# JingwenWang95/DSP-SLAM

Hardware: NVIDIA H100
Metric: object-recons/sec (2048 pts, 10 GN iters) (higher is better)
Workload: dtype f16x3-split (fp32 accumulate)

## Files before the change

### dsp_slam_b200/csrc/dspgn_tc.cuh

```cuda
#pragma once
#include <cuda_fp16.h>
#include <string>
#include <vector>
#include "dspgn_simt.cuh"
#include "dspgn_solve.cuh"

namespace dspgn {

constexpr int kTcThreads = 384;
constexpr int kTcEpiThreads = 256;
constexpr int kTcStages = 4;
constexpr int kTcStageBytes = 16384;
constexpr int kTcAloBytes = 32768;
constexpr int kTcProducerRegs = 40, kTcConsumerRegs = 232;
static_assert(128 * kTcProducerRegs + 256 * kTcConsumerRegs <= 384 * 168, "setmaxnreg budget exceeds the CTA's registers");

__host__ __device__ constexpr int tc_mma_n(int n) { return n <= 80 ? 80 : (n <= 192 ? 192 : 256); }
__host__ __device__ constexpr int tc_pad_k_steps(int k_steps) { return (k_steps + 3) / 4 * 4; }

__device__ __forceinline__ uint32_t smem_u32(const void* p) { return (uint32_t)__cvta_generic_to_shared(p); }

__device__ __forceinline__ void mbar_init(uint64_t* bar, uint32_t count) {
  asm volatile("mbarrier.init.shared::cta.b64 [%0], %1;" ::"r"(smem_u32(bar)), "r"(count) : "memory");
}
__device__ __forceinline__ void mbar_arrive(uint32_t bar) {
  asm volatile("mbarrier.arrive.shared::cta.b64 _, [%0];" ::"r"(bar) : "memory");
}
__device__ __forceinline__ void mbar_expect_tx(uint64_t* bar, uint32_t bytes) {
  asm volatile("mbarrier.arrive.expect_tx.shared::cta.b64 _, [%0], %1;" ::"r"(smem_u32(bar)), "r"(bytes) : "memory");
}
__device__ __forceinline__ void mbar_wait(uint32_t bar, uint32_t parity) {
  asm volatile(
      "{\n\t"
      ".reg .pred p;\n\t"
      "WAIT_LOOP:\n\t"
      "mbarrier.try_wait.parity.shared::cta.b64 p, [%0], %1;\n\t"
      "@p bra DONE;\n\t"
      "bra WAIT_LOOP;\n\t"
      "DONE:\n\t"
      "}" ::"r"(bar), "r"(parity) : "memory");
}
__device__ __forceinline__ void mbar_wait(uint64_t* bar, uint32_t parity) { mbar_wait(smem_u32(bar), parity); }
__device__ __forceinline__ void fence_barrier_init() { asm volatile("fence.mbarrier_init.release.cluster;" ::: "memory"); }

__device__ __forceinline__ void bulk_g2s(void* smem_dst, const void* gmem_src, uint32_t bytes, uint64_t* bar) {
  asm volatile("cp.async.bulk.shared::cluster.global.mbarrier::complete_tx::bytes [%0], [%1], %2, [%3];" ::"r"(smem_u32(smem_dst)),
               "l"(gmem_src), "r"(bytes), "r"(smem_u32(bar)) : "memory");
}

__device__ __forceinline__ void fence_proxy_async() { asm volatile("fence.proxy.async.shared::cta;" ::: "memory"); }
__device__ __forceinline__ void wg_fence() { asm volatile("wgmma.fence.sync.aligned;" ::: "memory"); }
__device__ __forceinline__ void wg_commit() { asm volatile("wgmma.commit_group.sync.aligned;" ::: "memory"); }
__device__ __forceinline__ void wg_wait0() { asm volatile("wgmma.wait_group.sync.aligned 0;" ::: "memory"); }
__device__ __forceinline__ void wg_wait1() { asm volatile("wgmma.wait_group.sync.aligned 1;" ::: "memory"); }
template <int REGS> __device__ __forceinline__ void setmaxnreg_inc() { asm volatile("setmaxnreg.inc.sync.aligned.u32 %0;" ::"n"(REGS)); }
template <int REGS> __device__ __forceinline__ void setmaxnreg_dec() { asm volatile("setmaxnreg.dec.sync.aligned.u32 %0;" ::"n"(REGS)); }
__device__ __forceinline__ void wg_bar_sync(int g) { asm volatile("bar.sync %0, 128;" ::"r"(3 + g) : "memory"); }

#define DSPGN_D8(o) "+f"(d[o + 0]), "+f"(d[o + 1]), "+f"(d[o + 2]), "+f"(d[o + 3]), "+f"(d[o + 4]), "+f"(d[o + 5]), "+f"(d[o + 6]), "+f"(d[o + 7])
#define DSPGN_D128                                                                                                    \
  DSPGN_D8(0), DSPGN_D8(8), DSPGN_D8(16), DSPGN_D8(24), DSPGN_D8(32), DSPGN_D8(40), DSPGN_D8(48), DSPGN_D8(56),         \
      DSPGN_D8(64), DSPGN_D8(72), DSPGN_D8(80), DSPGN_D8(88), DSPGN_D8(96), DSPGN_D8(104), DSPGN_D8(112), DSPGN_D8(120)
#define DSPGN_D96                                                                                                     \
  DSPGN_D8(0), DSPGN_D8(8), DSPGN_D8(16), DSPGN_D8(24), DSPGN_D8(32), DSPGN_D8(40), DSPGN_D8(48), DSPGN_D8(56),         \
      DSPGN_D8(64), DSPGN_D8(72), DSPGN_D8(80), DSPGN_D8(88)
#define DSPGN_D40 DSPGN_D8(0), DSPGN_D8(8), DSPGN_D8(16), DSPGN_D8(24), DSPGN_D8(32)
#define DSPGN_ACC_OPS128 "{%0, %1, %2, %3, %4, %5, %6, %7, %8, %9, %10, %11, %12, %13, %14, %15, %16, %17, %18, %19, %20, %21, %22, %23, %24, %25, %26, %27, %28, %29, %30, %31, %32, %33, %34, %35, %36, %37, %38, %39, %40, %41, %42, %43, %44, %45, %46, %47, %48, %49, %50, %51, %52, %53, %54, %55, %56, %57, %58, %59, %60, %61, %62, %63, %64, %65, %66, %67, %68, %69, %70, %71, %72, %73, %74, %75, %76, %77, %78, %79, %80, %81, %82, %83, %84, %85, %86, %87, %88, %89, %90, %91, %92, %93, %94, %95, %96, %97, %98, %99, %100, %101, %102, %103, %104, %105, %106, %107, %108, %109, %110, %111, %112, %113, %114, %115, %116, %117, %118, %119, %120, %121, %122, %123, %124, %125, %126, %127}, "
#define DSPGN_ACC_OPS96 "{%0, %1, %2, %3, %4, %5, %6, %7, %8, %9, %10, %11, %12, %13, %14, %15, %16, %17, %18, %19, %20, %21, %22, %23, %24, %25, %26, %27, %28, %29, %30, %31, %32, %33, %34, %35, %36, %37, %38, %39, %40, %41, %42, %43, %44, %45, %46, %47, %48, %49, %50, %51, %52, %53, %54, %55, %56, %57, %58, %59, %60, %61, %62, %63, %64, %65, %66, %67, %68, %69, %70, %71, %72, %73, %74, %75, %76, %77, %78, %79, %80, %81, %82, %83, %84, %85, %86, %87, %88, %89, %90, %91, %92, %93, %94, %95}, "
#define DSPGN_ACC_OPS40 "{%0, %1, %2, %3, %4, %5, %6, %7, %8, %9, %10, %11, %12, %13, %14, %15, %16, %17, %18, %19, %20, %21, %22, %23, %24, %25, %26, %27, %28, %29, %30, %31, %32, %33, %34, %35, %36, %37, %38, %39}, "

template <int N> struct Wgmma;
#define DSPGN_WGMMA(N, DREGS, OPS, R0, R1, R2, R3, R4, R5, S0, S1, S2)                                          \
  template <> struct Wgmma<N> {                                                                                 \
    static __device__ __forceinline__ void rs(float (&d)[128], uint32_t a0, uint32_t a1, uint32_t a2, uint32_t a3, \
                                              uint64_t b_desc) {                                                \
      asm volatile("{\n\t.reg .pred p;\n\tsetp.ne.b32 p, %" #R5 ", 0;\n\t"                                       \
                   "wgmma.mma_async.sync.aligned.m64n" #N "k16.f32.f16.f16 " OPS                                 \
                   "{%" #R0 ", %" #R1 ", %" #R2 ", %" #R3 "}, %" #R4 ", p, 1, 1, 0;\n\t}"                         \
                   : DREGS                                                                                      \
                   : "r"(a0), "r"(a1), "r"(a2), "r"(a3), "l"(b_desc), "r"(1)                                    \
                   : "memory");                                                                                 \
    }                                                                                                           \
    static __device__ __forceinline__ void ss(float (&d)[128], uint64_t a_desc, uint64_t b_desc) {              \
      asm volatile("{\n\t.reg .pred p;\n\tsetp.ne.b32 p, %" #S2 ", 0;\n\t"                                       \
                   "wgmma.mma_async.sync.aligned.m64n" #N "k16.f32.f16.f16 " OPS                                 \
                   "%" #S0 ", %" #S1 ", p, 1, 1, 0, 0;\n\t}"                                                     \
                   : DREGS                                                                                      \
                   : "l"(a_desc), "l"(b_desc), "r"(1)                                                           \
                   : "memory");                                                                                 \
    }                                                                                                           \
  };
DSPGN_WGMMA(256, DSPGN_D128, DSPGN_ACC_OPS128, 128, 129, 130, 131, 132, 133, 128, 129, 130)
DSPGN_WGMMA(192, DSPGN_D96, DSPGN_ACC_OPS96, 96, 97, 98, 99, 100, 101, 96, 97, 98)
DSPGN_WGMMA(80, DSPGN_D40, DSPGN_ACC_OPS40, 40, 41, 42, 43, 44, 45, 40, 41, 42)
#undef DSPGN_WGMMA

__device__ __forceinline__ void epi_bar_sync() { asm volatile("bar.sync 1, 256;" ::: "memory"); }

enum ProbeSlot {
  PR_WFULL, PR_WGWAIT, PR_GEMM, PR_EPI, PR_PROLOGUE, PR_JTJ, PR_TILE_END, PR_SOLVE, PR_FIFO, PR_LOOP, PR_TILES, PR_SOLVES,
  PR_WEMPTY, PR_POP, PR_PROD_LOOP, kProbeSlots = 16
};
constexpr int kProbeCtas = 256;
#ifdef DSPGN_STALL_PROBE
__device__ unsigned long long g_stall_probe[kProbeCtas * 3 * kProbeSlots];
__device__ __forceinline__ void probe_add(int slot, unsigned long long v) {
  if ((threadIdx.x & 127) == 0 && blockIdx.x < kProbeCtas)
    atomicAdd(&g_stall_probe[(blockIdx.x * 3 + (threadIdx.x >> 7)) * kProbeSlots + slot], v);
}
#define DSPGN_PROBE_T(t0) const long long t0 = clock64()
#define DSPGN_PROBE_ADD(slot, t0) probe_add(slot, (unsigned long long)(clock64() - (t0)))
#define DSPGN_PROBE_COUNT(slot) probe_add(slot, 1ull)
#else
#define DSPGN_PROBE_T(t0)
#define DSPGN_PROBE_ADD(slot, t0)
#define DSPGN_PROBE_COUNT(slot)
#endif

__device__ __forceinline__ uint64_t make_desc(uint32_t smem_addr) {
  uint64_t d = 0;
  d |= (uint64_t)((smem_addr >> 4) & 0x3FFF);
  d |= (uint64_t)1 << 16;
  d |= (uint64_t)64 << 32;
  d |= (uint64_t)1 << 62;
  return d;
}
__device__ __forceinline__ uint64_t make_desc_w(uint32_t smem_addr) {
  uint64_t d = 0;
  d |= (uint64_t)((smem_addr >> 4) & 0x3FFF);
  d |= (uint64_t)1 << 16;
  d |= (uint64_t)32 << 32;
  d |= (uint64_t)2 << 62;
  return d;
}

__device__ __forceinline__ void split_pack(float a, float b, uint32_t& hi, uint32_t& lo) {
  __half2 h = __floats2half2_rn(a, b);
  float2 back = __half22float2(h);
  __half2 l = __floats2half2_rn(a - back.x, b - back.y);
  hi = *reinterpret_cast<uint32_t*>(&h);
  lo = *reinterpret_cast<uint32_t*>(&l);
}

constexpr int kJpStride = 76;
struct TcSmemTail {
  float Jp[kTcRows * kJpStride];
  uint32_t maskw[8 * 4 * kTcEpiThreads];
  float bias[9 * kHid];
  float wlast[kHid];
  float w0x[3 * kHid];
  float zs[kMaxCode + 16];
  float xr[3 * kTcRows];
  float rr[kTcRows], rsc[kTcRows];
  float yrow[kTcRows], scr[kTcRows];
  int prefix[kMaxObjScan + 1];
  int warp_tmp[32];
  uint64_t w_full[kTcStages], w_empty[kTcStages];
  int cur_class;
  int fifo[4]; int fifo_pub; int epi_seq; int last_flag;
  TcPlan plans[DSPGN_MAX_CLASSES];
  BatchDev ctx_b; MegaArgs ctx_q; SolveArgs ctx_sv;
  int push_base, push_nF, push_nS, push_o;
  float ost[16]; int ost_rows;
};
constexpr size_t kTcSmemBytes = 1024 + (size_t)kTcStages * kTcStageBytes + 2 * (size_t)kTcAloBytes + sizeof(TcSmemTail);
static_assert(kTcSmemBytes <= 227 * 1024, "tensor-core engine shared memory exceeds the 227 KB per block of sm_90");
static_assert(offsetof(TcSmemTail, bias) % 8 == 0, "the hidden-layer epilogue reads bias column pairs as float2");

__device__ __forceinline__ int frag_col(int e, int q) { return 8 * (e >> 2) + 2 * q + (e & 1); }
__device__ __forceinline__ int opaque_int(int v) {
  int r;
  asm volatile("mov.b32 %0, %1;" : "=r"(r) : "r"(v));
  return r;
}

__device__ __forceinline__ void store_operand(const float (&v)[128], uint32_t (&ah)[64], unsigned char* alo, int rl, int q, int grp) {
#pragma unroll
  for (int t = 0; t < 16; ++t) {
#pragma unroll
    for (int h = 0; h < 4; ++h) {
      uint32_t hi, lo;
      split_pack(v[8 * t + 2 * h], v[8 * t + 2 * h + 1], hi, lo);
      ah[4 * t + h] = hi;
      const int row = rl + 8 * (h & 1), kk = 16 * t + 8 * (h >> 1) + 2 * q;
      const int off = (kk >> 6) * 8192 + row * 128 + ((((kk & 63) >> 3) ^ (row & 7)) << 4) + (kk & 7) * 2;
      *reinterpret_cast<uint32_t*>(alo + off) = lo;
    }
  }
  fence_proxy_async();
  wg_bar_sync(grp);
}

__device__ __forceinline__ void release_stage(uint32_t w_empty, int s) {
  __syncwarp();
  if ((threadIdx.x & 31) == 0) mbar_arrive(w_empty + 8u * s);
}

template <int N>
__device__ __forceinline__ void wg_gemm(float (&acc)[128], const uint32_t (&ah)[64], uint32_t alo, uint32_t ring,
                                        uint32_t bars, uint32_t& phase, int nch) {
  static_assert(kTcStages == 4, "one ring lap per K chunk");
  const uint32_t w_full = bars, w_empty = bars + 8u * kTcStages;
#pragma unroll
  for (int i = 0; i < 128; ++i) acc[i] = 0.f;
#pragma unroll
  for (int c = 0; c < 4; ++c) {
    if (c < nch) {
      const uint32_t ph = phase ^ (uint32_t)(c & 1);
#pragma unroll
      for (int s = 0; s < kTcStages; ++s) {
        DSPGN_PROBE_T(tf);
        mbar_wait(w_full + 8u * s, ph);
        DSPGN_PROBE_ADD(PR_WFULL, tf);
        wg_fence();
        const uint32_t bw = ring + (uint32_t)s * kTcStageBytes;
#pragma unroll
        for (int k = 0; k < 2; ++k) {
          const int t = 4 * c + 2 * (s & 1) + k;
          const uint64_t bd = make_desc_w(bw + 32u * k);
          Wgmma<N>::rs(acc, ah[4 * t], ah[4 * t + 1], ah[4 * t + 2], ah[4 * t + 3], bd);
          if (s < 2) Wgmma<N>::ss(acc, make_desc(alo + 8192u * c + 32u * (t & 3)), bd);
        }
        wg_commit();
        if (s == 1) {
          DSPGN_PROBE_T(tw);
          wg_wait1();
          DSPGN_PROBE_ADD(PR_WGWAIT, tw);
          release_stage(w_empty, 0);
          if (c > 0) release_stage(w_empty, 3);
        } else if (s == 3) {
          DSPGN_PROBE_T(tw);
          wg_wait1();
          DSPGN_PROBE_ADD(PR_WGWAIT, tw);
          release_stage(w_empty, 1);
          release_stage(w_empty, 2);
        }
      }
    }
  }
  DSPGN_PROBE_T(tw);
  wg_wait0();
  DSPGN_PROBE_ADD(PR_WGWAIT, tw);
  release_stage(w_empty, 3);
  phase ^= (uint32_t)(nch & 1);
}

__device__ __forceinline__ void produce_step(const unsigned char* src, int nch, uint32_t img_bytes, unsigned char* ring,
                                             uint64_t* w_full, uint64_t* w_empty, uint32_t& phase) {
  for (int c = 0; c < nch; ++c) {
    for (int s = 0; s < kTcStages; ++s) {
      DSPGN_PROBE_T(te);
      mbar_wait(&w_empty[s], phase ^ 1);
      DSPGN_PROBE_ADD(PR_WEMPTY, te);
      mbar_expect_tx(&w_full[s], img_bytes);
      bulk_g2s(ring + (size_t)s * kTcStageBytes, src + (size_t)(kTcStages * c + s) * img_bytes, img_bytes, &w_full[s]);
    }
    phase ^= 1;
  }
}

struct TileRef { int o, row0, slot, mode, tile; };

constexpr unsigned long long kMegaTimeoutNs = 30ull * 1000ull * 1000ull * 1000ull;
__device__ inline int mega_pop(const MegaArgs& q, int n_obj) {
  for (;;) {
    const int t = atomicAdd(&q.ctr->head, 1);
    if (t >= q.q_cap) return -1;
    unsigned long long t0 = 0;
    int item = kItemNop;
    for (unsigned spins = 0;; ++spins) {
      const int v = ldv(q.q_flag + t);
      if (v != 0) { __threadfence(); item = v - 1; break; }
      if (ldv(&q.ctr->done_objects) >= n_obj || ldv(&q.ctr->abort_flag) != 0) return -1;
      __nanosleep(256);
      if ((spins & 1023u) == 1023u) {
        const unsigned long long now = globaltimer_ns();
        if (t0 == 0) t0 = now;
        else if (now - t0 > kMegaTimeoutNs) { atomicExch(&q.ctr->abort_flag, 1); return -1; }
      }
    }
    if (item != kItemNop) return item;
  }
}

template <int SCHED>
__device__ __forceinline__ bool tile_at(const BatchDev& b, const TermArgs& a, TcSmemTail& S, int seq, int total_tiles, TileRef& t) {
  constexpr bool MEGA = SCHED != 0;
  if (!MEGA) {
    const int tile = blockIdx.x + seq * gridDim.x;
    if (tile >= total_tiles) return false;
    t.o = find_object(S.prefix, b.n_obj, tile);
    t.tile = tile - S.prefix[t.o];
    t.row0 = t.tile * kTcRows;
    t.slot = tile;
    t.mode = a.mode;
    return true;
  } else {
    volatile int* pub = &S.fifo_pub;
    while (*pub <= seq) __nanosleep(64);
    const int item = reinterpret_cast<volatile int*>(S.fifo)[seq & 3];
    if (item < 0) return false;
    t.o = (item >> kItemObjShift) & kItemObjMask;
    t.mode = (SCHED == 1) ? MODE_SDF : (item >> kItemKindShift);
    const int j = item & kItemTileMask;
    t.tile = j;
    t.row0 = j * kTcRows;
    t.slot = (t.mode == MODE_BAND) ? a.tile_base_r[t.o] + j : (t.mode == MODE_SDF ? a.tile_base[t.o] + j : 0);
    return true;
  }
}

__device__ __forceinline__ int mega_rows(const BatchDev& b, const MegaArgs& q, const ObjMeta& M, int o, int mode) {
  if (mode == MODE_SDF) return M.n_pts;
  if (mode == MODE_BAND) return ldv(b.band_m + o);
  if (q.vpre != nullptr) return ldv(q.vpre + vpre_base(M, o) + M.n_rays) >> 7;
  return M.n_rays * b.D;
}

__device__ inline void mega_push(const MegaArgs& q, int kind, int o, int n) {
  if (n <= 0) return;
  const int base = atomicAdd(&q.ctr->tail, n);
  __threadfence();
  for (int j = 0; j < n; ++j) *reinterpret_cast<volatile int*>(q.q_flag + base + j) = make_item(kind, o, j) + 1;
}

__device__ __noinline__ void mega_solve_and_advance(TcSmemTail& S, int o, int tid) {
  const BatchDev& b = S.ctx_b;
  const MegaArgs& q = S.ctx_q;
  const SolveArgs& sv = S.ctx_sv;
  __threadfence();
  SolveSmem& SM = *reinterpret_cast<SolveSmem*>(S.Jp);
  const int it = ldv(q.obj_iter + o);
  const bool render = q.render && b.state[o].mode == DSPGN_MODE_JOINT;
  if (tid == 0) log_event(q.log, ev_desc(EV_SOLVE_BEGIN, 0, o, it));
  const int fin = solve_object<true>(b, sv, q.log, o, tid, SM, it + 1 >= b.state[o].n_iter);
  epi_bar_sync();
  int vh = -1;
  if (!fin && render && q.vpre != nullptr) {
    const ObjMeta M = b.meta[o];
    if (M.n_rays > 0) vh = valid_sample_ranges<true>(M, b.state[o], b.rays, b.D, q.vpre + vpre_base(M, o), tid, kTcEpiThreads, S.warp_tmp);
  }
  if (tid == 0) {
    log_event(q.log, ev_desc(EV_SOLVE_END, 0, o, it));
// ... 86 lines not shown
        for (int s = 0; s < ns; ++s)
          produce_step(blob + plan.step[s].w_off, plan.step[s].k_steps / 4, 64u * (uint32_t)plan.step[s].n_mma, ring, S.w_full,
                       S.w_empty, phase);
      }
      DSPGN_PROBE_ADD(PR_PROD_LOOP, tloop);
    }
  } else {
    setmaxnreg_inc<kTcConsumerRegs>();
    const int grp = warp >> 2;
    const int r = tid & 127;
    const int qd = lane & 3;
    const int rl = 16 * (warp & 3) + (lane >> 2);
    const int rowA = 64 * grp + rl, rowB = rowA + 8;
    unsigned char* const alo = ring + (size_t)kTcStages * kTcStageBytes + (size_t)grp * kTcAloBytes;
    const uint32_t alo_s = smem_u32(alo), ring_s = smem_u32(ring);
    uint32_t phase = 0;
    float acc[128];
    uint32_t ah[64];
    DSPGN_PROBE_T(tloop);
    for (int seq = 0;; ++seq) {
      TileRef tr;
      DSPGN_PROBE_T(tq);
      if (!tile_at<SCHED>(b, a, S, seq, total_tiles, tr)) break;
      DSPGN_PROBE_ADD(PR_FIFO, tq);
      DSPGN_PROBE_T(tpro);
      if (MEGA && tid == 0) { *reinterpret_cast<volatile int*>(&S.epi_seq) = seq + 1; log_event(q.log, ev_desc(EV_TILE_BEGIN, tr.mode, tr.o, tr.tile)); }
      if (RENDER && tr.mode == kKindScan) {
        const int o = tr.o;
        scan_chunk(b, sv.prm.th, q.vpre, q.seg_cnt, o, tr.tile, tid);
        __threadfence();
        epi_bar_sync();
        if (tid == 0) {
          log_event(q.log, ev_desc(EV_TILE_END, tr.mode, o, tr.tile));
          *reinterpret_cast<volatile int*>(&S.last_flag) = (atomicSub(q.scan_left + o, 1) == 1) ? 1 : 0;
        }
        epi_bar_sync();
        int act = *reinterpret_cast<volatile int*>(&S.last_flag);
        if (act == 1) {
          __threadfence();
          scan_prefix(b, q.seg_cnt, q.seg_prefix, o, tid, S.warp_tmp);
          epi_bar_sync();
          if (tid == 0) {
            __threadfence();
            atomicAdd(&q.ctr->valid_rows_total, (unsigned long long)ldv(b.V_count + o));
            const int m = ldv(b.band_m + o);
            const int ntB = (m + kTcRows - 1) / kTcRows;
            atomicAdd(&q.ctr->band_rows_total, m);
            const int left = atomicAdd(q.pending + o, ntB - 1) + ntB - 1;
            mega_push(q, MODE_BAND, o, ntB);
            *reinterpret_cast<volatile int*>(&S.last_flag) = (left == 0) ? 2 : 0;
          }
          epi_bar_sync();
          act = *reinterpret_cast<volatile int*>(&S.last_flag);
        } else act = 0;
        if (act == 2) mega_solve_and_advance(S, o, tid);
        continue;
      }
      const int o = tr.o, row0 = tr.row0, tile = tr.slot, mode = tr.mode;
      const ObjMeta M = b.meta[o];
      const ObjState& ost = b.state[o];
      const DecoderDev& dec = b.decs[M.class_id];
      const TcPlan& plan = S.plans[M.class_id];
      const int L = dec.L, in0 = dec.in0, n_lin = dec.n_lin;
      const bool has_skip = dec.latent_in >= 0;
      const bool grid_mode = !MEGA && mode == MODE_GRIDFWD;
      const bool fwd_only = (mode == MODE_RAYFWD || mode == MODE_PTSFWD || grid_mode);
      const int ns = fwd_only ? plan.n_fwd : plan.n_steps;
      const float huber_b = term_huber(a, mode, ost.mode, (RENDER && mode == MODE_BAND) ? a.huber_b1 : a.huber_b);
      float* const part = (RENDER && mode == MODE_BAND) ? a.part_r : a.part;
      if (tid < 12) S.ost[tid] = ldv(&ost.T_oc[tid]);
      else if (tid < 16) S.ost[tid] = ldv(&ost.dmin + (tid - 12));
      const bool pts_mode = (mode == MODE_SDF || mode == MODE_PTSFWD || grid_mode);
      if (MEGA && !pts_mode && tid == 16) S.ost_rows = mega_rows(b, q, M, o, mode);

      if (S.cur_class != M.class_id) {
        for (int i = tid; i < n_lin * kHid; i += kTcEpiThreads) S.bias[i] = dec.bias[i / kHid][i % kHid];
        for (int i = tid; i < kHid; i += kTcEpiThreads) S.wlast[i] = dec.w_last[i];
        const float* __restrict__ w0g = dec.Wf[0] + (size_t)L * kHid;
        for (int i = tid; i < 3 * kHid; i += kTcEpiThreads) S.w0x[i] = w0g[i];
      }
      if (tid < kMaxCode + 16) S.zs[tid] = (tid < L) ? ldv(&ost.z[tid]) : 0.f;
      S.bias[tid] = ldv(&ost.zb0[tid]);
      const uint8_t* mask_in; uint8_t* mask_out;
      cut_masks(a, ost.mode, (MEGA && a.cut_iter >= 0) ? ldv(q.obj_iter + o) : a.iter, mask_in, mask_out);
      const int* segp = nullptr;
      int nseg = 0;
      const bool compact = RENDER && mode == MODE_RAYFWD && q.vpre != nullptr;
      if (compact) {
        int* sp = reinterpret_cast<int*>(S.Jp);
        const int* gp = q.vpre + vpre_base(M, o);
        for (int i = tid; i <= M.n_rays; i += kTcEpiThreads) sp[i] = __ldcg(gp + i);
        segp = sp;
      }
      if (RENDER && mode == MODE_BAND) {
        nseg = (M.n_rays + kSegRays - 1) / kSegRays;
        int* sp = reinterpret_cast<int*>(S.Jp);
        const int* gp = q.seg_prefix + seg_base(M, o);
        for (int i = tid; i <= nseg; i += kTcEpiThreads) sp[i] = __ldcg(gp + i);
        segp = sp;
      }
      int nrows = 0;
      float p0 = 0.f, p1 = 0.f, p2 = 0.f, sc = 0.f;
      if (pts_mode) {
        nrows = min(kTcRows, (MEGA ? M.n_pts : term_rows(b, a, o)) - row0);
        if (r < nrows) {
          const float* pq = grid_mode ? a.grid + 3 * (size_t)(row0 + r) : b.pts + 3 * (size_t)(M.pts_off + row0 + r);
          p0 = pq[0]; p1 = pq[1]; p2 = pq[2];
          sc = (grid_mode || mask_in == nullptr || ldv(mask_in + M.pts_off + row0 + r)) ? 1.f : 0.f;
        }
      }
      epi_bar_sync();
      float Toc[12];
#pragma unroll
      for (int i = 0; i < 12; ++i) Toc[i] = S.ost[i];
      if (!pts_mode) nrows = min(kTcRows, (MEGA ? S.ost_rows : term_rows(b, a, o)) - row0);
      float x0 = 0.f, x1 = 0.f, x2 = 0.f, res_in = 0.f;
      if (r < nrows) {
        const int rr_ = row0 + r;
        if (grid_mode) {
          x0 = p0; x1 = p1; x2 = p2;
        } else if (pts_mode) {
          xform_point(Toc, p0, p1, p2, x0, x1, x2);
        } else if (mode == MODE_BAND) {
          size_t sidx = (size_t)M.smp_off + rr_;
          if (RENDER) {
            int lo = 0, hi = nseg;
            while (hi - lo > 1) { const int mid = (lo + hi) >> 1; if (segp[mid] <= rr_) lo = mid; else hi = mid; }
            sidx = (size_t)M.smp_off + (size_t)lo * kSegRays * b.D + (size_t)(rr_ - segp[lo]);
          }
          x0 = __ldcg(b.band_x + 3 * sidx); x1 = __ldcg(b.band_x + 3 * sidx + 1); x2 = __ldcg(b.band_x + 3 * sidx + 2);
          sc = __ldcg(b.band_s + sidx); res_in = __ldcg(b.band_r + sidx);
        } else {
          int ray = rr_ / b.D, j = rr_ - ray * b.D;
          if (compact) {
            int lo = 0, hi = M.n_rays;
            while (hi - lo > 1) { const int mid = (lo + hi) >> 1; if ((segp[mid] >> 7) <= rr_) lo = mid; else hi = mid; }
            ray = lo; j = (segp[lo] & 127) + (rr_ - (segp[lo] >> 7));
          }
          const float* rq = b.rays + 3 * (size_t)(M.ray_off + ray);
          const float d = lin_depth(S.ost[12], S.ost[13], S.ost[14], j, b.D);
          xform_point(Toc, __fmul_rn(rq[0], d), __fmul_rn(rq[1], d), __fmul_rn(rq[2], d), x0, x1, x2);
          sc = inside_unit_sphere(x0, x1, x2) ? 1.f : 0.f;
        }
      }
      if (grp == 0) { S.xr[r] = x0; S.xr[kTcRows + r] = x1; S.xr[2 * kTcRows + r] = x2; S.scr[r] = sc; }
      epi_bar_sync();
      if (tid == 0) S.cur_class = M.class_id;

      auto inp = [&](int i, int row) -> float {
        const int j = i - L;
        return (j < 0) ? S.zs[i] : ((unsigned)j < 3u ? S.xr[j * kTcRows + row] : 0.f);
      };
      uint32_t* const maskw = S.maskw + tid;

      {
        const int kk = plan.step[0].k_steps * 16;
        const int n0out = dec.out_dim[0];
        const float* w0x = S.w0x;
        const float xa0 = S.xr[rowA], xa1 = S.xr[kTcRows + rowA], xa2 = S.xr[2 * kTcRows + rowA];
        const float xb0 = S.xr[rowB], xb1 = S.xr[kTcRows + rowB], xb2 = S.xr[2 * kTcRows + rowB];
        const int qs = opaque_int(qd);
        uint32_t mw[4] = {0u, 0u, 0u, 0u};
#pragma unroll
        for (int e = 0; e < 128; ++e) {
          const int c = frag_col(e, qs);
          const bool hb = (e & 2) != 0;
          float w = S.bias[c];
          w = fmaf(w0x[c], hb ? xb0 : xa0, w);
          w = fmaf(w0x[kHid + c], hb ? xb1 : xa1, w);
          w = fmaf(w0x[2 * kHid + c], hb ? xb2 : xa2, w);
          const bool on = (c < kk) && (c < n0out) && (w > 0.f);
          mw[e >> 5] |= (on ? 1u : 0u) << (e & 31);
          acc[e] = on ? w : 0.f;
        }
#pragma unroll
        for (int w = 0; w < 4; ++w) maskw[w * kTcEpiThreads] = mw[w];
        store_operand(acc, ah, alo, rl, qd, grp);
      }
      DSPGN_PROBE_ADD(PR_PROLOGUE, tpro);
      DSPGN_PROBE_COUNT(PR_TILES);

      float yv = 0.f;
      for (int s = 0; s < ns; ++s) {
        const TcStep st = plan.step[s];
        const bool more = (s + 1 < ns);
        const int k_next = more ? plan.step[s + 1].k_steps * 16 : 0;
        const int nm = st.n_mma;
        if (MEGA && tid == 0 && s == 0) log_event(q.log, ev_desc(EV_FIRST_MMA, tr.mode, tr.o, tr.tile));
        const int nch = st.k_steps / 4;
        DSPGN_PROBE_T(tg);
        if (nm == 80) wg_gemm<80>(acc, ah, alo_s, ring_s, smem_u32(S.w_full), phase, nch);
        else if (nm == 192) wg_gemm<192>(acc, ah, alo_s, ring_s, smem_u32(S.w_full), phase, nch);
        else wg_gemm<256>(acc, ah, alo_s, ring_s, smem_u32(S.w_full), phase, nch);
        DSPGN_PROBE_ADD(PR_GEMM, tg);
        DSPGN_PROBE_T(tepi);
        wg_bar_sync(grp);
        const int qs = opaque_int(qd);

        if (st.kind == TK_FWD_PENULT) {
          const float* bb = S.bias + st.layer * kHid;
          float pa = 0.f, pb = 0.f;
          uint32_t mw[4] = {0u, 0u, 0u, 0u};
#pragma unroll
          for (int e = 0; e < 128; ++e) {
            const int c = frag_col(e, qs);
            if (c < nm) {
              const float w = acc[e] + bb[c];
              mw[e >> 5] |= (w > 0.f ? 1u : 0u) << (e & 31);
              if (e & 2) pb = fmaf(fmaxf(w, 0.f), S.wlast[c], pb);
              else pa = fmaf(fmaxf(w, 0.f), S.wlast[c], pa);
            }
          }
#pragma unroll
          for (int w = 0; w < 4; ++w) maskw[(4 * st.layer + w) * kTcEpiThreads] = mw[w];
          pa += __shfl_xor_sync(0xffffffffu, pa, 1);
          pb += __shfl_xor_sync(0xffffffffu, pb, 1);
          pa += __shfl_xor_sync(0xffffffffu, pa, 2);
          pb += __shfl_xor_sync(0xffffffffu, pb, 2);
          const float blast = S.bias[(st.layer + 1) * kHid];
          const float ya = tanhf(pa + blast), yb = tanhf(pb + blast);
          if (qd == 0) { S.yrow[rowA] = ya; S.yrow[rowB] = yb; }
          epi_bar_sync();
          yv = S.yrow[r];
          if (fwd_only) {
            if (grp == 0 && r < nrows) {
              const size_t base = (mode == MODE_RAYFWD) ? (size_t)M.smp_off
                                  : (grid_mode ? (size_t)a.grid_slot[o] * a.grid_rows : (size_t)M.pts_off);
              b.sdf[base + row0 + r] = (sc != 0.f) ? yv : INFINITY;
            }
            if (!RENDER && mode == MODE_RAYFWD) {
              const unsigned bal = __ballot_sync(0xffffffffu, grp == 0 && r < nrows && sc != 0.f);
              if (lane == 0 && bal) atomicAdd(b.V_count + o, __popc(bal));
            }
          }
          if (more) {
            const float ga = 1.f - ya * ya, gb = 1.f - yb * yb;
#pragma unroll
            for (int e = 0; e < 128; ++e) {
              const int c = frag_col(e, qs);
              acc[e] = ((mw[e >> 5] >> (e & 31)) & 1u) ? ((e & 2) ? gb : ga) * S.wlast[c] : 0.f;
            }
            store_operand(acc, ah, alo, rl, qd, grp);
          }
        } else if (st.kind == TK_FWD_HIDDEN) {
          const float* bb = S.bias + st.layer * kHid;
          uint32_t mw[4] = {0u, 0u, 0u, 0u};
          if (SCHED == 1 && st.cat_off < 0) {
#pragma unroll
            for (int j = 0; j < 32; ++j) {
              const float2 bj = *reinterpret_cast<const float2*>(bb + 8 * j + 2 * qs);
#pragma unroll
              for (int h = 0; h < 4; ++h) {
                const int e = 4 * j + h, c = frag_col(e, qs);
                const float w = acc[e] + ((h & 1) ? bj.y : bj.x);
                const bool live = c < nm;
                mw[e >> 5] |= ((live && w > 0.f) ? 1u : 0u) << (e & 31);
                acc[e] = (live && c < k_next) ? fmaxf(w, 0.f) : 0.f;
              }
            }
          } else {
#pragma unroll
            for (int e = 0; e < 128; ++e) {
              const int c = frag_col(e, qs);
              float t = 0.f;
              if (c < nm) {
                const float w = acc[e] + bb[c];
                mw[e >> 5] |= (w > 0.f ? 1u : 0u) << (e & 31);
                t = fmaxf(w, 0.f);
              }
              if (st.cat_off >= 0 && c >= st.cat_off) t = inp(c - st.cat_off, (e & 2) ? rowB : rowA);
              acc[e] = (c < k_next) ? t : 0.f;
            }
          }
#pragma unroll
          for (int w = 0; w < 4; ++w) maskw[(4 * st.layer + w) * kTcEpiThreads] = mw[w];
          store_operand(acc, ah, alo, rl, qd, grp);
        } else if (st.kind == TK_BWD_MID) {
          uint32_t mw[4];
#pragma unroll
          for (int w = 0; w < 4; ++w) mw[w] = maskw[(4 * st.mask_layer + w) * kTcEpiThreads];
          if (SCHED == 1 && st.cat_off < 0) {
#pragma unroll
            for (int e = 0; e < 128; ++e) {
              const int c = frag_col(e, qs);
              const bool on = c < nm && c < k_next && ((mw[e >> 5] >> (e & 31)) & 1u);
              acc[e] = on ? acc[e] : 0.f;
            }
          } else {
#pragma unroll
            for (int e = 0; e < 128; ++e) {
              const int c = frag_col(e, qs);
              float t = 0.f;
              if (c < nm) {
                const float v = acc[e];
                t = ((mw[e >> 5] >> (e & 31)) & 1u) ? v : 0.f;
                if (st.cat_off >= 0 && c >= st.cat_off) {
                  const int ii = c - st.cat_off;
                  if (ii < in0) S.Jp[((e & 2) ? rowB : rowA) * kJpStride + ((ii < L) ? ii : (kMaxCode + ii - L))] = v;
                  t = 0.f;
                }
              }
              acc[e] = (c < k_next) ? t : 0.f;
            }
          }
          if (more) store_operand(acc, ah, alo, rl, qd, grp);
        } else {
#pragma unroll
          for (int e = 0; e < 128; ++e) {
            const int c = frag_col(e, qs);
            if (c < nm && c < in0) {
              const int row = (e & 2) ? rowB : rowA;
              float* pj = S.Jp + row * kJpStride + ((c < L) ? c : (kMaxCode + c - L));
              float g = acc[e];
              if (has_skip) g += *pj;
              *pj = g * S.scr[row];
            }
          }
        }
        if (!more || st.kind == TK_BWD_FIRST) {
#pragma unroll
          for (int i = 0; i < 64; ++i) ah[i] = 0u;
        }
        DSPGN_PROBE_ADD(PR_EPI, tepi);
      }
      DSPGN_PROBE_T(tjtj);
      if (!fwd_only) {
      epi_bar_sync();
      if (grp == 0) {
        float* jr = S.Jp + r * kJpStride;
        for (int i = L; i < kMaxCode; ++i) jr[i] = 0.f;
        const float g0 = jr[kMaxCode], g1 = jr[kMaxCode + 1], g2 = jr[kMaxCode + 2];
        jr[kMaxCode + 3] = x1 * g2 - x2 * g1;
        jr[kMaxCode + 4] = x2 * g0 - x0 * g2;
        jr[kMaxCode + 5] = x0 * g1 - x1 * g0;
        jr[kMaxCode + 6] = (ost.mode == DSPGN_MODE_POSE) ? 0.f : (g0 * x0 + g1 * x1 + g2 * x2);
        jr[kMaxCode + 7] = 0.f;
        float res = (mode == MODE_SDF) ? yv : res_in;
        if (sc == 0.f && (mode == MODE_SDF || r >= nrows)) res = 0.f;
        if (mask_out != nullptr && mode == MODE_SDF && r < nrows)
          mask_out[M.pts_off + row0 + r] = (sc != 0.f && fabsf(res) <= 0.05f) ? 1 : 0;
        S.rr[r] = huber_weight(fabsf(res), huber_b) * res;
        S.rsc[r] = (mode == MODE_SDF) ? sc : (r < nrows ? 1.f : 0.f);
        if (a.dbg_J != nullptr && o == a.dbg_obj && mode == MODE_SDF && r < nrows) a.dbg_res[row0 + r] = res;
      }
      epi_bar_sync();
      if (a.dbg_J != nullptr && o == a.dbg_obj && mode == MODE_SDF) {
        const int P = a.dbg_P, npose = (ost.mode == DSPGN_MODE_POSE) ? 6 : 7;
        for (int idx = tid; idx < nrows * P; idx += kTcEpiThreads) {
          const int p = idx / P, c = idx - p * P;
          const int ci = (c < npose) ? (kMaxCode + c) : (c - npose);
          a.dbg_J[(size_t)(row0 + p) * P + c] = S.Jp[p * kJpStride + ci];
        }
      }
      float* accp = part + (size_t)tile * kAccStride;
      if (tid < 171) {
        int bi = 0, rem = tid;
        while (rem >= 18 - bi) { rem -= 18 - bi; ++bi; }
        const int bj = bi + rem;
        float h[4][4];
#pragma unroll
        for (int u = 0; u < 4; ++u)
#pragma unroll
          for (int v = 0; v < 4; ++v) h[u][v] = 0.f;
        const float* pa = S.Jp + 4 * bi;
        const float* pb = S.Jp + 4 * bj;
#pragma unroll 4
        for (int p = 0; p < kTcRows; ++p) {
          const float4 A4 = *reinterpret_cast<const float4*>(pa + p * kJpStride);
          const float4 B4 = *reinterpret_cast<const float4*>(pb + p * kJpStride);
          const float av[4] = {A4.x, A4.y, A4.z, A4.w}, bv[4] = {B4.x, B4.y, B4.z, B4.w};
#pragma unroll
          for (int u = 0; u < 4; ++u)
#pragma unroll
            for (int v = 0; v < 4; ++v) h[u][v] = fmaf(av[u], bv[v], h[u][v]);
        }
#pragma unroll
        for (int u = 0; u < 4; ++u)
#pragma unroll
          for (int v = 0; v < 4; ++v) {
            const int rI = 4 * bi + u, cI = 4 * bj + v;
            if (cI >= rI && cI < kMaxCode + 7) accp[tri_index(rI, cI)] = h[u][v];
          }
      } else if (tid < 171 + kMaxCode + 7) {
        const int c = tid - 171;
        float sacc = 0.f;
        for (int p = 0; p < kTcRows; ++p) sacc = fmaf(S.Jp[p * kJpStride + c], S.rr[p], sacc);
        accp[kAccB + c] = sacc;
      } else if (tid >= 248) {
        const int k = tid - 248;
        float sacc = 0.f, n = 0.f;
        for (int p = 16 * k; p < 16 * k + 16; ++p) { sacc = fmaf(S.rr[p], S.rr[p], sacc); n += S.rsc[p]; }
#pragma unroll
        for (int d = 1; d < 8; d <<= 1) {
          sacc += __shfl_down_sync(0xff000000u, sacc, d);
          n += __shfl_down_sync(0xff000000u, n, d);
        }
        if (k == 0) { accp[kAccLoss] = sacc; accp[kAccLoss + 1] = n; }
      }
      }
      DSPGN_PROBE_ADD(PR_JTJ, tjtj);
      if (MEGA) {
        DSPGN_PROBE_T(tend);
        __threadfence();
        epi_bar_sync();
        if (tid == 0) {
          log_event(q.log, ev_desc(EV_TILE_END, mode, o, tr.tile));
          int act = 0;
          if (RENDER && mode == MODE_RAYFWD) { if (atomicSub(q.ray_left + o, 1) == 1) act = 1; }
          else if (atomicSub(q.pending + o, 1) == 1) act = 2;
          *reinterpret_cast<volatile int*>(&S.last_flag) = act;
        }
        epi_bar_sync();
        int act = *reinterpret_cast<volatile int*>(&S.last_flag);
        if (RENDER && act == 1) {
          if (tid == 0) {
            const int nch = (M.n_rays + kScanChunkRays - 1) / kScanChunkRays;
            *reinterpret_cast<volatile int*>(q.scan_left + o) = nch;
            __threadfence();
            mega_push(q, kKindScan, o, nch);
          }
        }
        DSPGN_PROBE_ADD(PR_TILE_END, tend);
        if (act == 2) {
          DSPGN_PROBE_T(tsv);
          mega_solve_and_advance(S, o, tid);
          DSPGN_PROBE_ADD(PR_SOLVE, tsv);
          DSPGN_PROBE_COUNT(PR_SOLVES);
        }
      }
    }
    DSPGN_PROBE_ADD(PR_LOOP, tloop);
  }
}

__global__ void __launch_bounds__(kTcThreads, 1) k_decoder_tc(BatchDev b, TermArgs a) {
  tc_body<0>(b, a, MegaArgs{}, SolveArgs{});
}
__global__ void __launch_bounds__(kTcThreads, 1) k_gn_persistent(BatchDev b, TermArgs a, MegaArgs q, SolveArgs sv) {
  tc_body<1>(b, a, q, sv);
}
__global__ void __launch_bounds__(kTcThreads, 1) k_gn_persistent_render(BatchDev b, TermArgs a, MegaArgs q, SolveArgs sv) {
  tc_body<2>(b, a, q, sv);
}

constexpr size_t kTcSelftestSmem = 1024 + (size_t)kTcStages * kTcStageBytes + 2 * (size_t)kTcAloBytes + 64;
__global__ void __launch_bounds__(kTcThreads, 1) k_tc_selftest(const float* __restrict__ A, int lda, const unsigned char* __restrict__ blob,
                                                               int n_mma, int k_steps, float* __restrict__ D) {
  extern __shared__ unsigned char st_raw[];
  unsigned char* ring = st_raw + ((1024u - (smem_u32(st_raw) & 1023u)) & 1023u);
  uint64_t* bars = reinterpret_cast<uint64_t*>(ring + (size_t)kTcStages * kTcStageBytes + 2 * (size_t)kTcAloBytes);
  uint64_t* w_full = bars;
  uint64_t* w_empty = bars + kTcStages;
  const int tid = threadIdx.x, warp = tid >> 5, lane = tid & 31;
  if (tid == 0) {
    for (int i = 0; i < kTcStages; ++i) { mbar_init(&w_full[i], 1); mbar_init(&w_empty[i], 8); }
    fence_barrier_init();
  }
  __syncthreads();
  const int n_img = tc_mma_n(n_mma), nch = tc_pad_k_steps(k_steps) / 4;
  uint32_t phase = 0;
  if (warp >= 8) {
    setmaxnreg_dec<kTcProducerRegs>();
    if (warp == 8 && lane == 0) produce_step(blob, nch, 64u * (uint32_t)n_img, ring, w_full, w_empty, phase);
    return;
  }
  setmaxnreg_inc<kTcConsumerRegs>();
  const int grp = warp >> 2, qd = lane & 3, rl = 16 * (warp & 3) + (lane >> 2);
  const int rowA = 64 * grp + rl, rowB = rowA + 8;
  unsigned char* alo = ring + (size_t)kTcStages * kTcStageBytes + (size_t)grp * kTcAloBytes;
  float acc[128];
// ... 137 lines not shown
```

Baseline: 4042.

## Specialize tensor-core epilogues and store low operand halves with stmatrix

For the SCHED==1 path, the low fp16 split halves are written to shared memory with stmatrix.x4 instead of per-element 32-bit stores. The per-kind epilogue loops (hidden forward, concat, skip gradient, backward mid, first backward) are rewritten to work on 8-column groups, with compile-time NM/KNEXT specializations for common widths, and the concat/skip layers now also take the fast path. The goal is fewer instructions, less predicate work and fewer shared-store transactions in the epilogue. The cost is more code paths and more register pressure, and the stmatrix swizzle has to match the existing layout exactly. Extra probe slots are also added for timing.

```diff
diff --git a/dsp_slam_b200/csrc/dspgn_tc.cuh b/dsp_slam_b200/csrc/dspgn_tc.cuh
--- a/dsp_slam_b200/csrc/dspgn_tc.cuh
+++ b/dsp_slam_b200/csrc/dspgn_tc.cuh
@@ -99,8 +99,9 @@
 
 enum ProbeSlot {
   PR_WFULL, PR_WGWAIT, PR_GEMM, PR_EPI, PR_PROLOGUE, PR_JTJ, PR_TILE_END, PR_SOLVE, PR_FIFO, PR_LOOP, PR_TILES, PR_SOLVES,
-  PR_WEMPTY, PR_POP, PR_PROD_LOOP, kProbeSlots = 16
+  PR_WEMPTY, PR_POP, PR_PROD_LOOP, PR_EPI_ENTRY, PR_EPI_KIND, kProbeSlots = PR_EPI_KIND + 3 * 6
 };
+enum EpiKind { EK_FWD, EK_FWD_CAT, EK_PENULT, EK_BWD, EK_BWD_SKIP, EK_BWD_FIRST };
 constexpr int kProbeCtas = 256;
 #ifdef DSPGN_STALL_PROBE
 __device__ unsigned long long g_stall_probe[kProbeCtas * 3 * kProbeSlots];
@@ -111,10 +112,12 @@
 #define DSPGN_PROBE_T(t0) const long long t0 = clock64()
 #define DSPGN_PROBE_ADD(slot, t0) probe_add(slot, (unsigned long long)(clock64() - (t0)))
 #define DSPGN_PROBE_COUNT(slot) probe_add(slot, 1ull)
+#define DSPGN_PROBE_ADD_IF(cond, slot, t0) do { if (cond) DSPGN_PROBE_ADD(slot, t0); } while (0)
 #else
 #define DSPGN_PROBE_T(t0)
 #define DSPGN_PROBE_ADD(slot, t0)
 #define DSPGN_PROBE_COUNT(slot)
+#define DSPGN_PROBE_ADD_IF(cond, slot, t0)
 #endif
 
 __device__ __forceinline__ uint64_t make_desc(uint32_t smem_addr) {
@@ -174,7 +177,9 @@
   return r;
 }
 
-__device__ __forceinline__ void store_operand(const float (&v)[128], uint32_t (&ah)[64], unsigned char* alo, int rl, int q, int grp) {
+__device__ __forceinline__ void store_operand(const float (&v)[128], uint32_t (&ah)[64], unsigned char* alo, int rl, int q, int grp,
+                                              int pslot = -1) {
+  DSPGN_PROBE_T(ts);
 #pragma unroll
   for (int t = 0; t < 16; ++t) {
 #pragma unroll
@@ -187,8 +192,109 @@
       *reinterpret_cast<uint32_t*>(alo + off) = lo;
     }
   }
+  DSPGN_PROBE_ADD_IF(pslot >= 0, pslot + 1, ts);
+  DSPGN_PROBE_T(tf);
   fence_proxy_async();
   wg_bar_sync(grp);
+  DSPGN_PROBE_ADD_IF(pslot >= 0, pslot + 2, tf);
+}
+
+__device__ __forceinline__ void store_operand_stsm(const float (&v)[128], uint32_t (&ah)[64], uint32_t alo, int grp, int pslot = -1) {
+  DSPGN_PROBE_T(ts);
+  const int lane = threadIdx.x & 31;
+  const int srow = 16 * ((threadIdx.x >> 5) & 3) + (lane & 7) + 8 * ((lane >> 3) & 1);
+  const uint32_t base = alo + 128u * (uint32_t)srow;
+  const uint32_t xo = (uint32_t)(((lane >> 4) & 1) ^ (lane & 7)) << 4;
+#pragma unroll
+  for (int t = 0; t < 16; ++t) {
+    uint32_t lo[4];
+#pragma unroll
+    for (int h = 0; h < 4; ++h) split_pack(v[8 * t + 2 * h], v[8 * t + 2 * h + 1], ah[4 * t + h], lo[h]);
+    const uint32_t addr = base + 8192u * (uint32_t)(t >> 2) + (xo ^ (32u * (uint32_t)(t & 3)));
+    asm volatile("stmatrix.sync.aligned.m8n8.x4.shared.b16 [%0], {%1, %2, %3, %4};" ::"r"(addr), "r"(lo[0]), "r"(lo[1]),
+                 "r"(lo[2]), "r"(lo[3]) : "memory");
+  }
+  DSPGN_PROBE_ADD_IF(pslot >= 0, pslot + 1, ts);
+  DSPGN_PROBE_T(tf);
+  fence_proxy_async();
+  wg_bar_sync(grp);
+  DSPGN_PROBE_ADD_IF(pslot >= 0, pslot + 2, tf);
+}
+
+template <int NM, int KNEXT>
+__device__ __forceinline__ void epi_fwd_hidden(float (&acc)[128], uint32_t (&mw)[4], const float* bb, int qs, int nm, int k_next) {
+#pragma unroll
+  for (int j = 0; j < 32; ++j) {
+    const bool live = 8 * j < (NM ? NM : nm), nxt = 8 * j < (KNEXT ? KNEXT : k_next);
+    const float2 bj = *reinterpret_cast<const float2*>(bb + 8 * j + 2 * qs);
+#pragma unroll
+    for (int h = 0; h < 4; ++h) {
+      const int e = 4 * j + h;
+      const float w = acc[e] + ((h & 1) ? bj.y : bj.x);
+      mw[e >> 5] |= ((live && w > 0.f) ? 1u : 0u) << (e & 31);
+      acc[e] = (live && nxt) ? fmaxf(w, 0.f) : 0.f;
+    }
+  }
+}
+
+__device__ __forceinline__ void epi_concat_input(float (&acc)[128], int qs, int k_next, int cat_off, int L, const float* zs,
+                                                 const float* xr, int rowA, int rowB) {
+#pragma unroll
+  for (int j = 0; j < 32; ++j) {
+    if (8 * j + 8 <= cat_off) continue;
+    const bool nxt = 8 * j < k_next;
+#pragma unroll
+    for (int h = 0; h < 4; ++h) {
+      const int e = 4 * j + h, i = 8 * j + 2 * qs + (h & 1) - cat_off, ix = i - L;
+      const float zv = zs[(unsigned)i < (unsigned)L ? i : 0];
+      const float xv = xr[((unsigned)ix < 3u ? ix : 0) * kTcRows + ((h & 2) ? rowB : rowA)];
+      acc[e] = (nxt && i >= 0) ? (i < L ? zv : ((unsigned)ix < 3u ? xv : 0.f)) : acc[e];
+    }
+  }
+}
+
+__device__ __forceinline__ void epi_skip_grad(float (&acc)[128], int qs, int nm, int cat_off, int in0, int L, float* Jp, int rowA,
+                                              int rowB) {
+#pragma unroll
+  for (int j = 0; j < 32; ++j) {
+    if (8 * j + 8 <= cat_off) continue;
+    const bool live = 8 * j < nm;
+#pragma unroll
+    for (int h = 0; h < 4; ++h) {
+      const int e = 4 * j + h, ii = 8 * j + 2 * qs + (h & 1) - cat_off;
+      if (live && ii >= 0 && ii < in0) Jp[((h & 2) ? rowB : rowA) * kJpStride + ((ii < L) ? ii : (kMaxCode + ii - L))] = acc[e];
+      acc[e] = (ii >= 0) ? 0.f : acc[e];
+    }
+  }
+}
+
+template <int NM, int KNEXT>
+__device__ __forceinline__ void epi_bwd_mid(float (&acc)[128], const uint32_t (&mw)[4], int nm, int k_next) {
+#pragma unroll
+  for (int j = 0; j < 32; ++j) {
+    const bool live = 8 * j < (NM ? NM : nm), nxt = 8 * j < (KNEXT ? KNEXT : k_next);
+#pragma unroll
+    for (int h = 0; h < 4; ++h) {
+      const int e = 4 * j + h;
+      acc[e] = (live && nxt && ((mw[e >> 5] >> (e & 31)) & 1u)) ? acc[e] : 0.f;
+    }
+  }
+}
+
+__device__ __forceinline__ void epi_bwd_first(const float (&acc)[128], int qs, int in0, int L, bool has_skip, float* Jp,
+                                              const float* scr, int rowA, int rowB) {
+  const float sa = scr[rowA], sb = scr[rowB];
+#pragma unroll
+  for (int j = 0; j < 10; ++j) {
+#pragma unroll
+    for (int h = 0; h < 4; ++h) {
+      const int c = 8 * j + 2 * qs + (h & 1);
+      const bool st = c < in0;
+      float* pj = Jp + ((h & 2) ? rowB : rowA) * kJpStride + (st ? ((c < L) ? c : (kMaxCode + c - L)) : 0);
+      const float g = has_skip ? acc[4 * j + h] + *pj : acc[4 * j + h];
+      if (st) *pj = g * ((h & 2) ? sb : sa);
+    }
+  }
 }
 
 __device__ __forceinline__ void release_stage(uint32_t w_empty, int s) {
@@ -581,6 +687,10 @@
         return (j < 0) ? S.zs[i] : ((unsigned)j < 3u ? S.xr[j * kTcRows + row] : 0.f);
       };
       uint32_t* const maskw = S.maskw + tid;
+      auto put_operand = [&](int pslot) {
+        if (SCHED == 1) store_operand_stsm(acc, ah, alo_s, grp, pslot);
+        else store_operand(acc, ah, alo, rl, qd, grp, pslot);
+      };
 
       {
         const int kk = plan.step[0].k_steps * 16;
@@ -604,7 +714,7 @@
         }
 #pragma unroll
         for (int w = 0; w < 4; ++w) maskw[w * kTcEpiThreads] = mw[w];
-        store_operand(acc, ah, alo, rl, qd, grp);
+        put_operand(-1);
       }
       DSPGN_PROBE_ADD(PR_PROLOGUE, tpro);
       DSPGN_PROBE_COUNT(PR_TILES);
@@ -624,6 +734,15 @@
         DSPGN_PROBE_ADD(PR_GEMM, tg);
         DSPGN_PROBE_T(tepi);
         wg_bar_sync(grp);
+        DSPGN_PROBE_ADD(PR_EPI_ENTRY, tepi);
+        DSPGN_PROBE_T(tval);
+#ifdef DSPGN_STALL_PROBE
+        const int pk = PR_EPI_KIND + 3 * (st.kind == TK_FWD_PENULT ? EK_PENULT
+                                          : st.kind == TK_FWD_HIDDEN ? (st.cat_off >= 0 ? EK_FWD_CAT : EK_FWD)
+                                          : st.kind == TK_BWD_MID ? (st.cat_off >= 0 ? EK_BWD_SKIP : EK_BWD) : EK_BWD_FIRST);
+#else
+        constexpr int pk = -1;
+#endif
         const int qs = opaque_int(qd);
 
         if (st.kind == TK_FWD_PENULT) {
@@ -669,24 +788,19 @@
               const int c = frag_col(e, qs);
               acc[e] = ((mw[e >> 5] >> (e & 31)) & 1u) ? ((e & 2) ? gb : ga) * S.wlast[c] : 0.f;
             }
-            store_operand(acc, ah, alo, rl, qd, grp);
+            DSPGN_PROBE_ADD(pk, tval);
+            put_operand(pk);
+          } else {
+            DSPGN_PROBE_ADD(pk, tval);
           }
         } else if (st.kind == TK_FWD_HIDDEN) {
           const float* bb = S.bias + st.layer * kHid;
           uint32_t mw[4] = {0u, 0u, 0u, 0u};
-          if (SCHED == 1 && st.cat_off < 0) {
-#pragma unroll
-            for (int j = 0; j < 32; ++j) {
-              const float2 bj = *reinterpret_cast<const float2*>(bb + 8 * j + 2 * qs);
-#pragma unroll
-              for (int h = 0; h < 4; ++h) {
-                const int e = 4 * j + h, c = frag_col(e, qs);
-                const float w = acc[e] + ((h & 1) ? bj.y : bj.x);
-                const bool live = c < nm;
-                mw[e >> 5] |= ((live && w > 0.f) ? 1u : 0u) << (e & 31);
-                acc[e] = (live && c < k_next) ? fmaxf(w, 0.f) : 0.f;
-              }
-            }
+          if (SCHED == 1) {
+            if (nm == 256 && k_next == 256) epi_fwd_hidden<256, 256>(acc, mw, bb, qs, nm, k_next);
+            else if (nm == 192 && k_next == 256) epi_fwd_hidden<192, 256>(acc, mw, bb, qs, nm, k_next);
+            else epi_fwd_hidden<0, 0>(acc, mw, bb, qs, nm, k_next);
+            if (st.cat_off >= 0) epi_concat_input(acc, qs, k_next, st.cat_off, L, S.zs, S.xr, rowA, rowB);
           } else {
 #pragma unroll
             for (int e = 0; e < 128; ++e) {
@@ -703,18 +817,17 @@
           }
 #pragma unroll
           for (int w = 0; w < 4; ++w) maskw[(4 * st.layer + w) * kTcEpiThreads] = mw[w];
-          store_operand(acc, ah, alo, rl, qd, grp);
+          DSPGN_PROBE_ADD(pk, tval);
+          put_operand(pk);
         } else if (st.kind == TK_BWD_MID) {
           uint32_t mw[4];
 #pragma unroll
           for (int w = 0; w < 4; ++w) mw[w] = maskw[(4 * st.mask_layer + w) * kTcEpiThreads];
-          if (SCHED == 1 && st.cat_off < 0) {
-#pragma unroll
-            for (int e = 0; e < 128; ++e) {
-              const int c = frag_col(e, qs);
-              const bool on = c < nm && c < k_next && ((mw[e >> 5] >> (e & 31)) & 1u);
-              acc[e] = on ? acc[e] : 0.f;
-            }
+          if (SCHED == 1) {
+            if (st.cat_off >= 0) epi_skip_grad(acc, qs, nm, st.cat_off, in0, L, S.Jp, rowA, rowB);
+            if (nm == 256 && k_next == 256) epi_bwd_mid<256, 256>(acc, mw, nm, k_next);
+            else if (nm == 256 && k_next == 192) epi_bwd_mid<256, 192>(acc, mw, nm, k_next);
+            else epi_bwd_mid<0, 0>(acc, mw, nm, k_next);
           } else {
 #pragma unroll
             for (int e = 0; e < 128; ++e) {
@@ -732,19 +845,25 @@
               acc[e] = (c < k_next) ? t : 0.f;
             }
           }
-          if (more) store_operand(acc, ah, alo, rl, qd, grp);
+          DSPGN_PROBE_ADD(pk, tval);
+          if (more) put_operand(pk);
         } else {
-#pragma unroll
-          for (int e = 0; e < 128; ++e) {
-            const int c = frag_col(e, qs);
-            if (c < nm && c < in0) {
-              const int row = (e & 2) ? rowB : rowA;
-              float* pj = S.Jp + row * kJpStride + ((c < L) ? c : (kMaxCode + c - L));
-              float g = acc[e];
-              if (has_skip) g += *pj;
-              *pj = g * S.scr[row];
+          if (SCHED == 1) {
+            epi_bwd_first(acc, qs, in0, L, has_skip, S.Jp, S.scr, rowA, rowB);
+          } else {
+#pragma unroll
+            for (int e = 0; e < 128; ++e) {
+              const int c = frag_col(e, qs);
+              if (c < nm && c < in0) {
+                const int row = (e & 2) ? rowB : rowA;
+                float* pj = S.Jp + row * kJpStride + ((c < L) ? c : (kMaxCode + c - L));
+                float g = acc[e];
+                if (has_skip) g += *pj;
+                *pj = g * S.scr[row];
+              }
             }
           }
+          DSPGN_PROBE_ADD(pk, tval);
         }
         if (!more || st.kind == TK_BWD_FIRST) {
 #pragma unroll
```

After: 4442 (median of 6 runs). +9.9%, better.
